# dcvan24/pivot-scheduling

Measured on AMD Instinct MI355X. Metric: task x host placement candidates scored/sec (HBM GB/s % peak) at 1/2/4/8 MI355X, higher is better.
Workload: dtype f64; 1 GPU; synthetic 1000000 hosts x 10000 ready tasks per round, 20 zones, cost_aware best-fit, one independent scenario per GPU; scenarios_per_gpu=1, tasks_per_round=10000, zones=20, policy=ca_bf, parallelism=scenario-sharded x1 (no data-path collective)

## Files before the change

pivot-scheduling_amd/csrc/pvt_capi.hip:

```cpp
#include <cstdarg>

#include "pvt_driver.h"
#include "pvt_opp.h"
#include "pvt_anchor.h"
#include "pvt_groups.h"
#include "pvt_meter.h"

int pvt::fail(pvt_ctx* c, int code, const char* fmt, ...) {
  char buf[512];
  va_list ap;
  va_start(ap, fmt);
  vsnprintf(buf, sizeof(buf), fmt, ap);
  va_end(ap);
  if (c) c->err = buf;
  return code;
}

int pvt::ensure(pvt_ctx* ctx, Buf& b, size_t bytes) {
  if (bytes == 0) bytes = 16;
  if (b.n >= bytes) return PVT_OK;
  const size_t want = std::max(bytes, b.n * 3 / 2);
  if (b.p) (void)hipFree(b.p);
  b.p = nullptr;
  b.n = 0;
// ... 182 lines not shown
extern "C" int pvt_reset_kstats(pvt_ctx* ctx) {
  if (!ctx) return PVT_EINVAL;
  (void)hipStreamSynchronize(ctx->stream);
  harvest(ctx);
  std::memset(ctx->ks, 0, sizeof(ctx->ks));
  ctx->kks.clear();
  return PVT_OK;
}
extern "C" int pvt_get_kstats(pvt_ctx* ctx, int kclass, pvt_kstats* out) {
  if (!ctx || !out || kclass < 0 || kclass >= PVT_K_COUNT) return PVT_EINVAL;
  (void)hipStreamSynchronize(ctx->stream);
  harvest(ctx);
  *out = ctx->ks[kclass];
  return PVT_OK;
}
extern "C" int pvt_get_kernel_kstats(pvt_ctx* ctx, const char* kernel, pvt_kstats* out) {
  if (!ctx || !kernel || !out) return PVT_EINVAL;
  (void)hipStreamSynchronize(ctx->stream);
  harvest(ctx);
  auto it = ctx->kks.find(kernel);
  if (it == ctx->kks.end()) std::memset(out, 0, sizeof(*out));
  else *out = it->second;
  return PVT_OK;
}
extern "C" int pvt_set_window(pvt_ctx* ctx, int tasks) {
  if (!ctx || tasks < 0) return PVT_EINVAL;
  ctx->window = std::min(tasks, MAX_WINDOW);
  return PVT_OK;
}
extern "C" int pvt_set_score_tw(pvt_ctx* ctx, int tw) {
  if (!ctx || (tw != 0 && tw != 2 && tw != 4)) return PVT_EINVAL;
  ctx->score_tw = tw;
  return PVT_OK;
}
extern "C" int pvt_set_pipeline(pvt_ctx* ctx, int on) {
  if (!ctx) return PVT_EINVAL;
  ctx->pipeline = on != 0;
  return PVT_OK;
}
extern "C" int pvt_set_epochs(pvt_ctx* ctx, int on) {
  if (!ctx) return PVT_EINVAL;
  ctx->epochs = on != 0;
  return PVT_OK;
}
extern "C" int pvt_epoch_stats(pvt_ctx* ctx, int64_t* epochs, int64_t* segments, int64_t* rejected) {
  if (!ctx) return PVT_EINVAL;
  if (epochs) *epochs = ctx->n_epochs;
  if (segments) *segments = ctx->n_segs;
  if (rejected) *rejected = ctx->n_rejected;
  return PVT_OK;
}
extern "C" int pvt_set_band(pvt_ctx* ctx, int32_t min_hosts) {
  if (!ctx || min_hosts < 0) return PVT_EINVAL;
  ctx->band_min = min_hosts;
  return PVT_OK;
}
extern "C" int pvt_set_zero_walk(pvt_ctx* ctx, int on) {
  if (!ctx) return PVT_EINVAL;
  ctx->zwalk = on != 0;
  return PVT_OK;
}
extern "C" int pvt_zero_walk_stats(pvt_ctx* ctx, int64_t* frontier_chains, int64_t* list_chains,
                                   int64_t* longest_chain) {
  if (!ctx) return PVT_EINVAL;
  if (frontier_chains) *frontier_chains = ctx->n_zchains;
  if (list_chains) *list_chains = ctx->n_gchains;
  if (longest_chain) *longest_chain = ctx->n_longest;
  return PVT_OK;
}
extern "C" int pvt_prologue_stats(pvt_ctx* ctx, int64_t* fast_chains) {
  if (!ctx) return PVT_EINVAL;
  if (fast_chains) *fast_chains = ctx->n_fastpro;
  return PVT_OK;
}
extern "C" int pvt_last_stats(pvt_ctx* ctx, int64_t* windows, int64_t* refills) {
  if (!ctx) return PVT_EINVAL;
  if (windows) *windows = ctx->windows;
  if (refills) *refills = ctx->refills;
  return PVT_OK;
}
extern "C" int pvt_debug_commit_stamps(pvt_ctx* ctx, uint64_t* out, int n) {
  if (!ctx || !out || n < 8) return PVT_EINVAL;
#ifdef PVT_STAMPS
  constexpr int NW = 32 + 4096;
  if (!ctx->stamps) {
    if (hipMalloc((void**)&ctx->stamps, sizeof(uint64_t) * NW) != hipSuccess) return PVT_ENOMEM;
    (void)hipMemset(ctx->stamps, 0, sizeof(uint64_t) * NW);
    std::memset(out, 0, sizeof(uint64_t) * std::min(n, NW));
    return PVT_OK;
  }
  if (hipMemcpy(out, ctx->stamps, sizeof(uint64_t) * std::min(n, NW), hipMemcpyDeviceToHost) != hipSuccess)
    return PVT_EHIP;
  return PVT_OK;
#else
  return PVT_EUNSUPPORTED;
#endif
}

extern "C" int pvt_debug_score_counts(pvt_ctx* ctx, uint64_t* out, int n, int reset) {
  if (!ctx || !out || n < 5) return PVT_EINVAL;
  (void)hipSetDevice(ctx->device);
  return pvt::score_diag(out, n, reset);
}

static_assert(PVT_MAX_ZONES == pvt::ZWIDE, "the public zone bound is the wide kernels' bound");
extern "C" int pvt_max_zones(void) { return PVT_MAX_ZONES; }

extern "C" const char* pvt_last_error(pvt_ctx* ctx) { return ctx ? ctx->err.c_str() : "null context"; }

int pvt::check_round(pvt_ctx* ctx, const pvt_round* r) {
  if (!r) return fail(ctx, PVT_EINVAL, "null round");
  if (r->reserved != 0) return fail(ctx, PVT_EINVAL, "reserved must be 0");
  if (r->n_hosts < 1 || r->n_tasks < 0 || r->n_zones < 1 || r->n_zones > PVT_MAX_ZONES)
    return fail(ctx, PVT_EINVAL, "bad sizes H=%d T=%d Z=%d (1 <= Z <= PVT_MAX_ZONES = %d)", r->n_hosts,
                r->n_tasks, r->n_zones, PVT_MAX_ZONES);
  if (r->mode < PVT_CA_FF || r->mode > PVT_VBP_BF) return fail(ctx, PVT_EINVAL, "bad mode %d", r->mode);
  if (!r->avail || !r->zone) return fail(ctx, PVT_EINVAL, "null host array");
  if (r->n_tasks > 0 && (!r->dem || !r->order || !r->placement))
    return fail(ctx, PVT_EINVAL, "null task array");
  if ((r->mode == PVT_CA_FF || r->mode == PVT_CA_BF) && (!r->cost || !r->bw))
    return fail(ctx, PVT_EINVAL, "cost_aware needs cost and bw");
  if (r->n_tasks > 0 && r->task_group && (r->n_groups < 1 || !r->group_anchor))
    return fail(ctx, PVT_EINVAL, "task_group needs n_groups >= 1 and group_anchor");
  if (r->mode == PVT_VBP_BF && !r->tiebreak) return fail(ctx, PVT_EINVAL, "vbp best-fit needs tiebreak");
  if (r->mode == PVT_OPP && !r->mt_state) return fail(ctx, PVT_EINVAL, "opportunistic needs mt_state");
  if (r->mode == PVT_CA_BF && r->decay && r->n_tasks > 0)
    return fail(ctx, PVT_EUNSUPPORTED, "cost_aware best-fit with host_decay (reference crashes, cost_aware.py:26,81)");
  return PVT_OK;
}

static const char* const CHK_NAMES[CHK_RULES + 1] = {
    "ok", "zone", "avail", "dem", "task_group", "group_anchor", "cost", "bw", "rt_bw", "decay",
    "tiebreak", "mt_state"};

int pvt::fail_check(pvt_ctx* ctx, int i, const pvt_check_report& p) {
  char where[32] = "";
  if (i >= 0) std::snprintf(where, sizeof(where), "round %d: ", i);
  return fail(ctx, PVT_EINVAL, "%scheck failed: rule %d (%s) at index %lld, value %.17g (%lld "
              "violating, mask 0x%x)", where, p.code, CHK_NAMES[p.code], (long long)p.index, p.value,
              (long long)p.count, (unsigned)p.mask);
}

static void check_mtpos(const pvt_round* r, pvt_check_report* p) {
  if (r->mode != PVT_OPP || !r->mt_state || !chk_bad_mtpos(r->mt_state[624])) return;
  p->mask |= 1 << PVT_CHK_MTPOS;
  if (p->code) return;
  p->code = PVT_CHK_MTPOS;
  p->index = 624;
  p->count = 1;
  p->value = (double)r->mt_state[624];
}

void pvt::check_host_arrays(const pvt_round* r, pvt_check_report* p) {
  check_on_host(check_describe(*r), p);
  check_mtpos(r, p);
}

static int run_checks(pvt_ctx* ctx, const pvt_round* rounds, int n, pvt_check_report* out,
                      bool host_mt) {
  for (int i = 0; i < n; i++) {
    int rc = check_round(ctx, &rounds[i]);
    if (rc) return rc;
  }
  HIPCHK(hipSetDevice(ctx->device));
  hipStream_t st = ctx->stream;
  std::vector<CheckRound>& cr = ctx->chk_host;
  cr.resize(n);
// ... 169 lines not shown
```

pivot-scheduling_amd/csrc/pvt_kernels.h:

```cpp
#pragma once
#include <hip/hip_runtime.h>
#include <hip/hip_ext.h>
#include <stdint.h>

namespace pvt {

struct TimedEvents {
  hipEvent_t a = nullptr, b = nullptr;
  bool armed = false;
  int used = 0, extra = 0;
};
extern thread_local TimedEvents g_timed;
#define PVT_LAUNCH(kernel, grid, block, shmem, stream, ...)                                         \
  do {                                                                                             \
    ::pvt::TimedEvents& te_ = ::pvt::g_timed;                                                      \
    if (te_.armed && te_.a) {                                                                      \
      hipExtLaunchKernelGGL(kernel, grid, block, shmem, stream, te_.a, te_.b, 0u, __VA_ARGS__);    \
      te_.a = nullptr;                                                                             \
      te_.used++;                                                                                  \
    } else {                                                                                       \
      if (te_.armed) te_.extra++;                                                                  \
      hipLaunchKernelGGL(kernel, grid, block, shmem, stream, __VA_ARGS__);                         \
    }                                                                                              \
  } while (0)
// ... 413 lines not shown
              resident_switches(32, 1025) == resident_switches(32, 1024), "32 holds at every size");
static_assert(resident_switches(64 + (12 << 8), 1024) == ResidentSwitches{0, 0, 0, 0, 1, 1, 1, 12} &&
              resident_switches(64 + (12 << 8), 1025) == resident_switches(64 + (12 << 8), 1024),
              "64 and the list minimum hold at every size");
static_assert(resident_switches(2, 1024) == ResidentSwitches{1, 0, 1, 1, 1, 1, 0, 0}, "2: rotated walker");
struct ResidentArgs {
  const void* rounds;
  uint32_t* mt;
  int Zb;
  int Tpad;
  uint64_t* stamps;
  ResidentSwitches sw;
};
size_t resident_lds_bytes(int Zb, int Tpad, const ResidentSwitches& sw);
void resident_shape(int maxH, int* waves, int* hpl);
void launch_resident(int mode, int waves, int hpl, int n, size_t lds, const ResidentArgs& a,
                     hipStream_t st);
hipError_t resident_init_attrs();
constexpr int RES_WIDE_MAX_HPL = 8;
constexpr int RES_WIDE_MAX_HOSTS = 4 * WAVE * RES_WIDE_MAX_HPL;
void launch_resident_wide(int mode, int hpl, int n, size_t lds, const ResidentArgs& a, hipStream_t st);
hipError_t resident_wide_init_attrs();

struct FusedRound {
  int64_t out_lo, out_hi, in_lo, in_hi;
  int64_t desc;
  int32_t items, pad;
};
struct FusedArgs {
  const char* hmap;
  char* dev;
  int64_t o_rounds;
  int64_t o_ka, o_kg;
  ResidentArgs ra;
};
size_t fused_pre_lds_bytes();
void launch_fused(int mode, int hpl, int n, size_t lds, const FusedArgs& F, hipStream_t st);
void launch_fused_wide(int mode, int hpl, int n, size_t lds, const FusedArgs& F, hipStream_t st);
size_t commit_lds_bytes();
hipError_t init_kernel_attrs();
constexpr int GSORT_MAX = 4096;
void launch_group_hist(const int32_t* tg, int T, int G, int32_t* cnt, hipStream_t st);
constexpr int PREP_T_MAX = 65536;
constexpr int GAGG_MAX = 4096;
struct PrepArgs {
  const int32_t* tg;
  int T, G;
  const int32_t* ganc;
  const double* cost;
  const double* bw;
  int Z, nz2;
  const double* dem;
  int sort_tasks;
  int32_t* placement;
  int32_t* off;
  int32_t* hcnt;
  int32_t* hgan;
  double* hcst;
  double* csum;
  double* bsum;
  uint64_t* skey;
  int32_t* sidx;
  int32_t* hflag;
  int32_t seq;
};
void launch_order_prep(const PrepArgs& a, hipStream_t st, hipEvent_t counted = nullptr,
                       bool scatter = true);
constexpr int GCOMPACT_MAX = 64;
struct GatherOut {
  int32_t* ord;
  double* dem_ord;
  int32_t* anc_ord;
  int32_t* grp_ord;
  int32_t* order_out;
  const double* avail;
  int H;
  double* hmin;
  uint64_t* stamps;
  const int32_t* zone;
  struct ZoneWindows* zwin;
  struct GroupCert* gcert;
};
static_assert(GC_SUB * 64 == GSORT_MAX, "a group record holds every sub-batch of a sorted group");
void launch_group_sort_gather(const PrepArgs& a, const GatherOut& o, hipStream_t st);
void launch_upload(const void* src_mapped, void* dst, size_t bytes, hipStream_t st);
void launch_restore_hosts(double* avail, const double* avail0, int H, const int32_t* hosts, int n,
                          hipStream_t st);
void launch_group_stage(const int32_t* cnt, int G, const int32_t* ganc, const double* cost, int nz2,
                        int32_t* off, int32_t* hcnt, int32_t* hgan, double* hcst, hipStream_t st);
void launch_group_scatter(const int32_t* tg, const uint64_t* keys, int T, int G, int32_t* cursor,
                          uint64_t* skey, int32_t* sidx, hipStream_t st);
void launch_group_sort(const int32_t* off, int G, const uint64_t* skey, const int32_t* sidx,
                       int32_t* ord, hipStream_t st);
void launch_iota(int32_t* out, int n, hipStream_t st);
void launch_gather_tasks(const double* dem, const int32_t* ord, const int32_t* task_group,
                         const int32_t* group_anchor, int T, double* dem_ord, int32_t* anc_ord,
                         int32_t* grp_ord, hipStream_t st, int G = 0x7fffffff,
                         int32_t* order_out = nullptr);

}
```

pivot-scheduling_amd/csrc/pvt_kernels.hip:

```cpp
#include <hip/hip_runtime.h>
#include <algorithm>
#include <stdint.h>
#include <stdlib.h>

#include "pvt_device.h"
#include "pvt_kernels.h"
#include "pvt_zwin_dev.h"
#include "pvt_list.h"

namespace pvt {

#ifdef PVT_DIAG
__device__ unsigned long long g_score_diag[8];
#endif

template <int MODE, int TWP>
__global__ __launch_bounds__(256) void score_kernel(ScoreArgs A) {
  constexpr bool WIDE = TWP < 0;
  constexpr int TW = WIDE ? -TWP : TWP;
  constexpr bool STRICT = (MODE != CA_BF);
  constexpr int ZL = (MODE == CA_BF && !WIDE) ? ZMAX : 1;
  __shared__ double s_lim[WPB][TW][ZL];
  __shared__ double s_rad[WPB][TW][ZL];
  __shared__ double s_c[WPB][TW][ZL];
// ... 996 lines not shown
  __threadfence_system();
  if (A.hflag) {
    __syncthreads();
    if (t == 0) {
      __hip_atomic_store(A.hflag, A.seq, __ATOMIC_RELEASE, __HIP_MEMORY_SCOPE_SYSTEM);
    }
  }
}
__global__ __launch_bounds__(1024) void order_count_kernel(PrepArgs A) {
  __shared__ int32_t cnt[GAGG_MAX + 1];
  order_count_body(A, cnt);
}

__global__ __launch_bounds__(1024) void order_scatter_kernel(PrepArgs A) {
  __shared__ int32_t cur[GAGG_MAX];
  __shared__ int32_t wsum[16];
  __shared__ int32_t carry;
  const int t = threadIdx.x, lane = t & 63, wave = t >> 6;
  const int T = A.T, G = A.G;
  if (t == 0) carry = 0;
  if (A.placement)
    for (int i = t; i < T; i += 1024) A.placement[i] = -1;
  if (A.csum)
    for (int i = t; i < A.Z * A.Z; i += 1024) {
      const int a = i / A.Z, z = i - a * A.Z;
      A.csum[i] = A.cost[a * A.Z + z] + A.cost[z * A.Z + a];
      A.bsum[i] = A.bw[a * A.Z + z] + A.bw[z * A.Z + a];
    }
  __syncthreads();
  for (int g0 = 0; g0 < G; g0 += 1024) {
    const int g = g0 + t;
    const int v = g < G ? A.off[g] : 0;
    int x = v;
#pragma unroll
    for (int o = 1; o < 64; o <<= 1) {
      const int y = __shfl_up(x, o);
      if (lane >= o) x += y;
    }
    if (lane == 63) wsum[wave] = x;
    __syncthreads();
    int pre = carry;
    for (int w = 0; w < wave; w++) pre += wsum[w];
    if (g < G) { A.off[g] = pre + x - v; cur[g] = pre + x - v; }
    __syncthreads();
    if (t == 1023) carry = pre + x;
    __syncthreads();
  }
  if (t == 0) A.off[G] = carry;
  constexpr int PS = 8;
  for (int i0 = 0; i0 < T; i0 += 1024 * PS) {
    int gv[PS];
    double dv[PS][4];
#pragma unroll
    for (int u = 0; u < PS; u++) {
      const int i = i0 + u * 1024 + t;
      gv[u] = i < T ? A.tg[i] : -1;
      if (A.sort_tasks && i < T) {
        dv[u][0] = A.dem[i]; dv[u][1] = A.dem[(size_t)T + i];
        dv[u][2] = A.dem[2 * (size_t)T + i]; dv[u][3] = A.dem[3 * (size_t)T + i];
      }
    }
#pragma unroll
    for (int u = 0; u < PS; u++) {
      const int i = i0 + u * 1024 + t;
      const int g = gv[u];
      if (i >= T || g < 0 || g >= G) continue;
      uint64_t key = 0;
      if (A.sort_tasks) {
        const double n = __builtin_sqrt(norm2_seq(dv[u][0], dv[u][1], dv[u][2], dv[u][3]));
        key = ~(uint64_t)__double_as_longlong(n);
      }
      const int pos = atomicAdd(&cur[g], 1);
      A.skey[pos] = key;
      A.sidx[pos] = i;
    }
  }
}
void launch_order_prep(const PrepArgs& a, hipStream_t st, hipEvent_t counted, bool scatter) {
  PVT_LAUNCH(order_count_kernel, dim3(1), dim3(1024), 0, st, a);
  if (counted) (void)hipEventRecord(counted, st);
  if (scatter) PVT_LAUNCH(order_scatter_kernel, dim3(1), dim3(1024), 0, st, a);
}

__device__ void lds_sort_pairs(uint64_t* k, int32_t* v, int n) {
  const int tid = threadIdx.x;
  if (n <= 128) {
    int r = 0;
    int32_t vi = 0;
    if (tid < n) {
      const uint64_t ki = k[tid];
      vi = v[tid];
      for (int j = 0; j < n; j++) {
        const uint64_t kj = k[j];
        r += (kj < ki || (kj == ki && v[j] < vi)) ? 1 : 0;
      }
    }
    __syncthreads();
    if (tid < n) v[r] = vi;
    __syncthreads();
    return;
  }
  int P = 2;
  while (P < n) P <<= 1;
  constexpr int EMAX = GSORT_MAX / 1024;
  const int E = (P + 1023) >> 10;
  uint64_t rk[EMAX];
  int32_t rv[EMAX];
#pragma unroll
  for (int m = 0; m < EMAX; m++) {
    const int i = m * 1024 + tid;
    rk[m] = (m < E && i < n) ? k[i] : ~0ull;
    rv[m] = (m < E && i < n) ? v[i] : (0x40000000 + i);
  }
  __syncthreads();
  const int P64 = min(P, 64);
  for (int size = 2; size <= P64; size <<= 1) {
    for (int stride = size >> 1; stride > 0 && (tid & ~63) < P; stride >>= 1) {
#pragma unroll
      for (int m = 0; m < EMAX; m++) {
        if (m >= E) continue;
        const int i = m * 1024 + tid;
        const uint32_t klo = (uint32_t)rk[m], khi = (uint32_t)(rk[m] >> 32);
        const uint64_t pk = ((uint64_t)(uint32_t)__shfl_xor((int)khi, stride) << 32) |
                            (uint32_t)__shfl_xor((int)klo, stride);
        const int32_t pv = __shfl_xor(rv[m], stride);
        const bool up = size == P64 || (i & size) == 0, low = (i & stride) == 0;
        const uint64_t kl = low ? rk[m] : pk, kh = low ? pk : rk[m];
        const int32_t vl = low ? rv[m] : pv, vh = low ? pv : rv[m];
        const bool gt = kl > kh || (kl == kh && vl > vh);
        if (gt == up) { rk[m] = pk; rv[m] = pv; }
      }
    }
  }
  if (P <= 64) {
#pragma unroll
    for (int m = 0; m < EMAX; m++) {
      const int i = m * 1024 + tid;
      if (m < E && i < n) v[i] = rv[m];
    }
    __syncthreads();
    return;
  }
  __shared__ uint64_t k2[GSORT_MAX];
  __shared__ int32_t v2[GSORT_MAX];
#pragma unroll
  for (int m = 0; m < EMAX; m++) {
    const int i = m * 1024 + tid;
    if (m < E && i < P) { k[i] = rk[m]; v[i] = rv[m]; }
  }
  __syncthreads();
  uint64_t* ka = k;
  int32_t* va = v;
  uint64_t* kb = k2;
  int32_t* vb = v2;
  for (int w = 64; w < P; w <<= 1) {
#pragma unroll
    for (int m = 0; m < EMAX; m++) {
      const int i = m * 1024 + tid;
      if (m >= E || i >= P) continue;
      const uint64_t key = ka[i];
      const int32_t val = va[i];
      const int base = i & ~(2 * w - 1), off = i - base;
      const bool left = off < w;
      const int ob = left ? base + w : base;
      int lo = 0, len = w;
      while (len > 0) {
        const int half = len >> 1, mid = lo + half;
        const uint64_t km = ka[ob + mid];
        const bool below = km < key || (km == key && va[ob + mid] < val);
        lo = below ? mid + 1 : lo;
        len = below ? len - half - 1 : half;
      }
      const int dest = base + (left ? off : off - w) + lo;
      kb[dest] = key;
      vb[dest] = val;
    }
    __syncthreads();
    uint64_t* tk = ka; ka = kb; kb = tk;
    int32_t* tv = va; va = vb; vb = tv;
  }
  if (va != v) {
    for (int i = tid; i < n; i += 1024) v[i] = va[i];
    __syncthreads();
  }
}

__global__ __launch_bounds__(1024) void group_sort_kernel(const int32_t* off, const uint64_t* skey,
                                                          const int32_t* sidx, int32_t* ord) {
  __shared__ uint64_t k[GSORT_MAX];
  __shared__ int32_t v[GSORT_MAX];
  const int a = off[blockIdx.x], n = off[blockIdx.x + 1] - a, tid = threadIdx.x;
  if (n <= 0 || n > GSORT_MAX) return;
  for (int i = tid; i < n; i += blockDim.x) { k[i] = skey[a + i]; v[i] = sidx[a + i]; }
  __syncthreads();
  lds_sort_pairs(k, v, n);
  for (int i = tid; i < n; i += blockDim.x) ord[a + i] = v[i];
}

__device__ void zone_window_block(const PrepArgs& A, const GatherOut& O, int j, int32_t* lds) {
  __shared__ uint32_t am[ZMAX], reach[ZMAX], gm_s;
  __shared__ int32_t cnt[2][16], nw_s;
  const int tid = threadIdx.x, Z = A.Z;
  ZoneWindows* W = O.zwin;
  if (tid < ZMAX) am[tid] = 0;
  if (tid == 0) { gm_s = 0; nw_s = 0; }
  __syncthreads();
  for (int i = tid; i < Z * Z; i += 1024) {
    const int a = i / Z, z = i - a * Z;
    if (A.cost[a * Z + z] + A.cost[z * Z + a] == 0.0) atomicOr(&am[a], 1u << z);
  }
  for (int g = tid; g < A.G; g += 1024) {
    const int a = A.ganc[g];
    if (a >= 0 && a < Z) atomicOr(&gm_s, 1u << a);
  }
  __syncthreads();
  if (tid < Z) reach[tid] = am[tid] | (1u << tid);
  __syncthreads();
  for (int it = 0; it < 5; it++) {
    uint32_t r = 0;
    if (tid < Z) {
      r = reach[tid];
      for (uint32_t m = r; m; m &= m - 1) r |= reach[__builtin_ctz(m)];
    }
    __syncthreads();
    if (tid < Z) reach[tid] = r;
    __syncthreads();
  }
  const uint32_t comp = reach[j];
  uint32_t U = 0;
  if ((comp & ((1u << j) - 1u)) == 0)
    for (uint32_t m = comp & gm_s; m; m &= m - 1) U |= am[__builtin_ctz(m)];
  if (tid == 0) W->U[j] = U;
  if (U == 0) return;
  int32_t* wid = lds;
  int32_t* wz = lds + ZW_M;
  compact_zone_window_t<ZW_M, 1024, 2>(O.zone, Z, U, 0, O.H, wid, wz, cnt, &nw_s);
  const int n = nw_s;
  ZoneWindow& w = W->w[j];
  bool bad = false;
  for (int p = tid; p < n; p += 1024) {
    const int h = wid[p];
    w.id[p] = h;
    w.z[p] = wz[p];
#pragma unroll
    for (int r = 0; r < 4; r++) {
      const double x = O.avail[(size_t)r * O.H + h];
      bad |= !(__builtin_fabs(x) <= 0x1p500);
      w.a[r][p] = x;
    }
  }
  bad = __syncthreads_or(bad);
  if (tid == 0) { w.n = n; w.bad = bad ? 1 : 0; }
}

#ifdef PVT_STAMPS
__device__ __forceinline__ uint64_t gstamp() {
  uint64_t t;
  __builtin_amdgcn_sched_barrier(0);
  asm volatile("s_memtime %0\n\ts_waitcnt lgkmcnt(0)" : "=s"(t)::"memory");
  __builtin_amdgcn_sched_barrier(0);
  return t;
}
#define GSTAMP(k) do { if (g == 0 && tid == 0 && O.stamps) { const uint64_t t_ = gstamp(); gph[k] = t_ - gtl; gtl = t_; } } while (0)
#else
#define GSTAMP(k) do {} while (0)
#endif

__global__ __launch_bounds__(1024) void group_sort_gather_kernel(PrepArgs A, GatherOut O) {
  __shared__ uint64_t k[GSORT_MAX];
  __shared__ int32_t v[GSORT_MAX];
  __shared__ int32_t fill, below_s;
  static_assert(sizeof(k) >= sizeof(int32_t) * (GCOMPACT_MAX + 1), "count table in k");
  if (blockIdx.x == 0) {
    order_count_body(A, reinterpret_cast<int32_t*>(k));
    return;
  }
  const int g = blockIdx.x - 1, tid = threadIdx.x, lane = tid & 63;
  const int T = A.T;
#ifdef PVT_STAMPS
  uint64_t gph[4] = {0, 0, 0, 0}, gtl = 0;
  if (g == 0 && tid == 0) gtl = gstamp();
#endif
  const int nmin = O.hmin ? ZW_MIN_PARTS : 0;
  if (g >= A.G + nmin) {
    zone_window_block(A, O, g - A.G - nmin, reinterpret_cast<int32_t*>(k));
    return;
  }
  if (g >= A.G) {
    __shared__ double red[16][4];
    const int pb = g - A.G, wave = tid >> 6;
    double m[4] = {DINF, DINF, DINF, DINF};
    constexpr int STEP = ZW_MIN_PARTS * 1024;
    for (int h0 = pb * 1024 + tid; h0 < O.H; h0 += 4 * STEP) {
      double x[4][4];
#pragma unroll
      for (int j = 0; j < 4; j++) {
        const int h = h0 + j * STEP;
#pragma unroll
        for (int r = 0; r < 4; r++) x[j][r] = h < O.H ? O.avail[(size_t)r * O.H + h] : DINF;
      }
#pragma unroll
      for (int j = 0; j < 4; j++)
#pragma unroll
        for (int r = 0; r < 4; r++) m[r] = fmin(m[r], x[j][r]);
    }
#pragma unroll
    for (int r = 0; r < 4; r++) {
      for (int off = 32; off > 0; off >>= 1) m[r] = fmin(m[r], __shfl_xor(m[r], off));
      if (lane == 0) red[wave][r] = m[r];
    }
    __syncthreads();
    if (tid < 4) {
      double x = red[0][tid];
      for (int w = 1; w < 16; w++) x = fmin(x, red[w][tid]);
      O.hmin[pb * 4 + tid] = x;
    }
    return;
  }
  if (g == 0 && A.csum)
    for (int i = tid; i < A.Z * A.Z; i += 1024) {
      const int a = i / A.Z, z = i - a * A.Z;
      A.csum[i] = A.cost[a * A.Z + z] + A.cost[z * A.Z + a];
      A.bsum[i] = A.bw[a * A.Z + z] + A.bw[z * A.Z + a];
    }
  if (tid == 0) { fill = 0; below_s = 0; }
  __syncthreads();
  GSTAMP(0);
  const uint64_t below = (lane == 0) ? 0ull : (~0ull >> (64 - lane));
  constexpr int PB = 8;
  for (int i0 = 0; i0 < T; i0 += 1024 * PB) {
    int gv[PB];
#pragma unroll
    for (int u = 0; u < PB; u++) {
      const int i = i0 + u * 1024 + tid;
      gv[u] = i < T ? A.tg[i] : -1;
    }
    uint64_t bal[PB];
    int tot = 0, lt = 0;
#pragma unroll
    for (int u = 0; u < PB; u++) {
      const int i = i0 + u * 1024 + tid;
      const bool mine = gv[u] == g;
      if (mine && A.placement) A.placement[i] = -1;
      bal[u] = __ballot(mine);
      tot += __popcll(bal[u]);
      lt += __popcll(__ballot(gv[u] >= 0 && gv[u] < g));
    }
    if (lane == 0 && lt) atomicAdd(&below_s, lt);
    if (tot == 0) continue;
    int b = 0;
    if (lane == 0) b = atomicAdd(&fill, tot);
    b = __shfl(b, 0);
    if (b + tot > GSORT_MAX) continue;
#pragma unroll
    for (int u = 0; u < PB; u++) {
      if (gv[u] == g) v[b + __popcll(bal[u] & below)] = i0 + u * 1024 + tid;
      b += __popcll(bal[u]);
    }
  }
  __syncthreads();
  const int n = fill;
  if (n > GSORT_MAX && tid == 0 && O.gcert) { O.gcert[g].bad = 2; O.gcert[g].n = n; }
  if (n > GSORT_MAX || n <= 0) return;
  for (int q = tid; q < n; q += 1024) {
    uint64_t key = 0;
    if (A.sort_tasks) {
      const int i = v[q];
      const double nn = __builtin_sqrt(norm2_seq(A.dem[i], A.dem[(size_t)T + i],
                                                 A.dem[2 * (size_t)T + i], A.dem[3 * (size_t)T + i]));
      key = ~(uint64_t)__double_as_longlong(nn);
    }
    k[q] = key;
  }
  __syncthreads();
  GSTAMP(1);
  lds_sort_pairs(k, v, n);
  GSTAMP(2);
  const int a = below_s;
  const int32_t anc = A.ganc[g];
  GroupCert* const gc = O.gcert ? O.gcert + g : nullptr;
  const int wave = __builtin_amdgcn_readfirstlane(tid >> 6);
  double gmx[4] = {-DINF, -DINF, -DINF, -DINF}, gmn[4] = {DINF, DINF, DINF, DINF};
  bool gbad = false;
  for (int i0 = 0; i0 < n; i0 += 1024) {
    const int i = i0 + tid;
    double d[4] = {0.0, 0.0, 0.0, 0.0};
    if (i < n) {
      const int p = a + i, t = v[i];
      O.ord[p] = t;
      if (O.order_out) O.order_out[p] = t;
      double* o = O.dem_ord + (size_t)p * 4;
      d[0] = A.dem[t]; d[1] = A.dem[(size_t)T + t]; d[2] = A.dem[2 * (size_t)T + t]; d[3] = A.dem[3 * (size_t)T + t];
      o[0] = d[0]; o[1] = d[1]; o[2] = d[2]; o[3] = d[3];
      O.anc_ord[p] = anc;
      O.grp_ord[p] = g;
    }
    if (gc && i0 + wave * 64 < n) {
#pragma unroll
      for (int r = 0; r < 4; r++) {
        const double f = readlane_d(d[r], 0);
        const double x = i < n ? d[r] : f;
        gbad |= !(__builtin_fabs(x) <= 0x1p500);
        gmx[r] = fmax(gmx[r], x);
        double m = f;
        if (__ballot(__double_as_longlong(x) != __double_as_longlong(f)) != 0) m = wave_min_d(x);
        gmn[r] = fmin(gmn[r], m);
        if (lane == 0) gc->smin[(i0 >> 6) + wave][r] = m;
      }
    }
  }
  if (gc) {
    double* red = reinterpret_cast<double*>(k);
#pragma unroll
    for (int r = 0; r < 4; r++) {
      const double f = readlane_d(gmx[r], 0);
      double m = f;
      if (__ballot(__double_as_longlong(gmx[r]) != __double_as_longlong(f)) != 0) m = wave_max_d(gmx[r]);
      if (lane == 0) { red[wave * 8 + r] = m; red[wave * 8 + 4 + r] = gmn[r]; }
    }
    gbad = __syncthreads_or(gbad);
    if (tid < 8) {
      double x = red[tid];
      for (int w = 1; w < 16; w++) x = tid < 4 ? fmax(x, red[w * 8 + tid]) : fmin(x, red[w * 8 + tid]);
      if (tid < 4) gc->mx[tid] = x; else gc->mn[tid - 4] = x;
    }
    if (tid == 0) { gc->bad = gbad ? 1 : 0; gc->n = n; }
  }
#ifdef PVT_STAMPS
  __syncthreads();
  GSTAMP(3);
  if (g == 0 && tid == 0 && O.stamps)
    for (int q = 0; q < 4; q++) atomicAdd((unsigned long long*)&O.stamps[16 + q], (unsigned long long)gph[q]);
#endif
}
void launch_group_sort_gather(const PrepArgs& a, const GatherOut& o, hipStream_t st) {
  const int extra = (o.hmin ? ZW_MIN_PARTS : 0) + (o.zwin ? a.Z : 0);
  PVT_LAUNCH(group_sort_gather_kernel, dim3(1 + a.G + extra), dim3(1024), 0, st, a, o);
}
void launch_group_sort(const int32_t* off, int G, const uint64_t* skey, const int32_t* sidx,
                       int32_t* ord, hipStream_t st) {
  PVT_LAUNCH(group_sort_kernel, dim3(G), dim3(1024), 0, st, off, skey, sidx, ord);
}

__global__ __launch_bounds__(256) void restore_hosts_kernel(double* avail, const double* avail0, int H,
                                                            const int32_t* hosts, int n) {
  const int i = blockIdx.x * 256 + threadIdx.x;
  if (i >= n) return;
  const int h = hosts[i];
  if (h < 0 || h >= H) return;
#pragma unroll
  for (int r = 0; r < 4; r++) avail[(size_t)r * H + h] = avail0[(size_t)r * H + h];
}
void launch_restore_hosts(double* avail, const double* avail0, int H, const int32_t* hosts, int n,
                          hipStream_t st) {
  if (n > 0) PVT_LAUNCH(restore_hosts_kernel, dim3((n + 255) / 256), dim3(256), 0, st, avail, avail0, H, hosts, n);
}

__global__ __launch_bounds__(256) void upload_kernel(const int4* src, int4* dst, int n16) {
  for (int i = blockIdx.x * 256 + threadIdx.x; i < n16; i += gridDim.x * 256) dst[i] = src[i];
}
void launch_upload(const void* src_mapped, void* dst, size_t bytes, hipStream_t st) {
  const int n16 = (int)((bytes + 15) / 16);
  if (n16 <= 0) return;
  const int blocks = std::min(64, (n16 + 255) / 256);
  PVT_LAUNCH(upload_kernel, dim3(blocks), dim3(256), 0, st,
                     reinterpret_cast<const int4*>(src_mapped), reinterpret_cast<int4*>(dst), n16);
}

__global__ void iota_kernel(int32_t* out, int n) {
  const int i = blockIdx.x * blockDim.x + threadIdx.x;
  if (i < n) out[i] = i;
}
void launch_iota(int32_t* out, int n, hipStream_t st) {
  PVT_LAUNCH(iota_kernel, dim3((n + 255) / 256), dim3(256), 0, st, out, n);
}

__global__ void gather_tasks_kernel(const double* dem, const int32_t* ord, const int32_t* tg,
                                    const int32_t* ga, int T, double* dem_ord, int32_t* anc_ord,
                                    int32_t* grp_ord, int G, int32_t* order_out) {
  const int p = blockIdx.x * blockDim.x + threadIdx.x;
  if (p >= T) return;
  const int t = ord[p];
  if (order_out) order_out[p] = t;
  double* o = dem_ord + (size_t)p * 4;
  o[0] = dem[t]; o[1] = dem[(size_t)T + t]; o[2] = dem[2 * (size_t)T + t]; o[3] = dem[3 * (size_t)T + t];
  if (anc_ord) anc_ord[p] = (tg && ga && tg[t] >= 0 && tg[t] < G) ? ga[tg[t]] : 0;
  if (grp_ord) grp_ord[p] = tg ? tg[t] : 0;
}
void launch_gather_tasks(const double* dem, const int32_t* ord, const int32_t* task_group,
                         const int32_t* group_anchor, int T, double* dem_ord, int32_t* anc_ord,
                         int32_t* grp_ord, hipStream_t st, int G, int32_t* order_out) {
  PVT_LAUNCH(gather_tasks_kernel, dim3((T + 255) / 256), dim3(256), 0, st, dem, ord,
                     task_group, group_anchor, T, dem_ord, anc_ord, grp_ord, G, order_out);
}

}
```

pivot-scheduling_amd/csrc/pvt_round.hip:

```cpp
#include <hipcub/hipcub.hpp>

#include <limits>

#include "pvt_driver.h"
#include "pvt_opp.h"
#include "pvt_groups.h"

static constexpr size_t SEG_ENTRIES_MAX = (size_t)MAX_WINDOW * MAX_SEG * KL;
static int choose_segments(int H, int nt, int mode, int force_tw, bool epoch, int force_S, int Z) {
  const int tw = score_tasks_per_wave(mode, H, force_tw, Z);
  const int task_waves = (nt + tw - 1) / tw;
  int S = (4096 + task_waves - 1) / task_waves;
  if (mode == PVT_VBP_BF) S = std::min(S, 16);
  if (mode == PVT_CA_BF && epoch) S = 4;
  if (force_S > 0) S = force_S;
  S = std::min(S, std::max(1, H / 4096));
  S = std::min(S, std::max(MAX_SEG, (int)(SEG_ENTRIES_MAX / ((size_t)nt * KL))));
  S = std::max(1, std::min(S, 256));
  if (S >= 8) S = S / 8 * 8;
  return S;
}
static constexpr int KSCAN_DEPTH = 256;
static constexpr int KPREFIX_MIN = 1024;
double pvt::bytes_per_candidate(int mode) {
// ... 7 lines not shown
    if (n >= (1u << 18)) {
      HIPCHK(hipStreamSynchronize(ctx->stream));
      if (__atomic_load_n(f, __ATOMIC_ACQUIRE) == seq) return PVT_OK;
      return fail(ctx, PVT_EHIP, "%s: kernel finished without its flag", what);
    }
    if ((n & 4095) == 0) {
      const hipError_t e = hipStreamQuery(ctx->stream);
      if (e == hipSuccess) {
        if (__atomic_load_n(f, __ATOMIC_ACQUIRE) == seq) return PVT_OK;
        return fail(ctx, PVT_EHIP, "%s: kernel finished without its flag", what);
      }
      if (e != hipErrorNotReady) return fail(ctx, PVT_EHIP, "%s: %s", what, hipGetErrorString(e));
    }
  }
}
static int wait_stage_flag(pvt_ctx* ctx) {
  return wait_host_flag(ctx, ctx->flag_host, ctx->flag_seq, "grouped order");
}

static int build_order_radix(pvt_ctx* ctx, const pvt_round* r, int32_t** ord_out);
static int build_order(pvt_ctx* ctx, const pvt_round* r, int32_t** ord_out, bool* pending,
                       double* hmin = nullptr, bool* hmin_done = nullptr,
                       ZoneWindows* zwin = nullptr) {
  *pending = false;
  if (hmin_done) *hmin_done = false;
  ctx->rs.stage_flag = false;
  const int T = r->n_tasks;
  hipStream_t st = ctx->stream;
  ENSURE(ctx->ord, sizeof(int32_t) * T);
  ENSURE(ctx->ord2, sizeof(int32_t) * T);
  int32_t* cur = P<int32_t>(ctx->ord);
  const bool grouped = r->task_group != nullptr && r->n_groups > 1;
  RoundState& R = ctx->rs;
  R.ginfo = false;
  R.zpre = false;
  R.gcert = false;
  if (grouped && r->n_groups <= (1 << 20)) {
    const int G = r->n_groups;
    const bool fused = T <= PREP_T_MAX && G <= GAGG_MAX;
    if (!fused) {
      ENSURE(ctx->gcnt, sizeof(int32_t) * (G + 1));
      HIPCHK(hipMemsetAsync(ctx->gcnt.p, 0, sizeof(int32_t) * (G + 1), st));
      launch_group_hist(r->task_group, T, G, P<int32_t>(ctx->gcnt), st);
    }
    const bool ca = r->mode == PVT_CA_FF || r->mode == PVT_CA_BF;
    const size_t nz2 = ca ? (size_t)r->n_zones * r->n_zones : 0;
    const size_t need = sizeof(double) * nz2 + sizeof(int32_t) * (2 * (size_t)G + 1);
    if (ctx->gstage_cap < need) {
      if (ctx->gstage) (void)hipHostFree(ctx->gstage);
      ctx->gstage = nullptr;
      ctx->gstage_cap = 0;
      HIPCHK(hipHostMalloc(&ctx->gstage, need));
      ctx->gstage_cap = need;
    }
    ENSURE(ctx->goff, sizeof(int32_t) * 2 * (G + 1));
    void* dstage = nullptr;
    HIPCHK(hipHostGetDevicePointer(&dstage, ctx->gstage, 0));
    double* dcst = reinterpret_cast<double*>(dstage);
    int32_t* dcnt = reinterpret_cast<int32_t*>(dcst + nz2);
    ENSURE(ctx->gskey, sizeof(uint64_t) * T);
    ENSURE(ctx->gsidx, sizeof(int32_t) * T);
    if (fused) {
      if (ca) {
        ENSURE(ctx->csum, sizeof(double) * r->n_zones * r->n_zones);
        ENSURE(ctx->bsum, sizeof(double) * r->n_zones * r->n_zones);
      }
      PrepArgs pa{r->task_group, T, G, r->group_anchor, r->cost, r->bw, r->n_zones, (int)nz2,
                  r->dem, r->sort_tasks ? 1 : 0, r->placement, P<int32_t>(ctx->goff), dcnt,
                  dcnt + G + 1, dcst, ca ? P<double>(ctx->csum) : nullptr,
                  ca ? P<double>(ctx->bsum) : nullptr, P<uint64_t>(ctx->gskey), P<int32_t>(ctx->gsidx),
                  nullptr, 0};
      R.prep_fused = true;
      if (G <= GCOMPACT_MAX) {
        pa.hflag = ctx->flag_hdev;
        pa.seq = ++ctx->flag_seq;
        R.stage_flag = true;
        const bool zw = hmin && zwin && ca && r->n_zones <= ZMAX;
        const bool gc = zw && ctx->t_chain_cert;
        if (gc) ENSURE(ctx->gcert, sizeof(GroupCert) * (size_t)GCOMPACT_MAX);
        launch_group_sort_gather(pa, GatherOut{cur, P<double>(ctx->dem_ord), P<int32_t>(ctx->anc_ord),
                                               P<int32_t>(ctx->grp_ord), r->order, r->avail,
                                               r->n_hosts, hmin, ctx->stamps, r->zone,
                                               zw ? zwin : nullptr,
                                               gc ? P<GroupCert>(ctx->gcert) : nullptr}, st);
        if (hmin_done) *hmin_done = hmin != nullptr;
        R.zpre = zw;
        R.gcert = gc;
        R.gathered = true;
        R.ginfo = ca;
        *pending = true;
        *ord_out = cur;
        return PVT_OK;
      }
      launch_order_prep(pa, st, ctx->ev_stage);
    } else {
      launch_group_stage(P<int32_t>(ctx->gcnt), G, r->group_anchor, r->cost, (int)nz2,
                         P<int32_t>(ctx->goff), dcnt, dcnt + G + 1, dcst, st);
      HIPCHK(hipGetLastError());
      const uint64_t* keys = nullptr;
      if (r->sort_tasks) {
        ENSURE(ctx->keys64a, sizeof(uint64_t) * T);
        launch_norm_keys(r->dem, T, nullptr, P<uint64_t>(ctx->keys64a), st);
        keys = P<uint64_t>(ctx->keys64a);
      }
      launch_group_scatter(r->task_group, keys, T, G, P<int32_t>(ctx->goff) + G + 1,
                           P<uint64_t>(ctx->gskey), P<int32_t>(ctx->gsidx), st);
      HIPCHK(hipEventRecord(ctx->ev_stage, st));
    }
    launch_group_sort(P<int32_t>(ctx->goff), G, P<uint64_t>(ctx->gskey), P<int32_t>(ctx->gsidx),
                      cur, st);
    R.ginfo = ca;
    *pending = true;
    *ord_out = cur;
    return PVT_OK;
  }
  return build_order_radix(ctx, r, ord_out);
}

static int build_order_check(pvt_ctx* ctx, const pvt_round* r, bool* redo) {
  RoundState& R = ctx->rs;
  const int G = r->n_groups;
  const bool ca = r->mode == PVT_CA_FF || r->mode == PVT_CA_BF;
  const size_t nz2 = ca ? (size_t)r->n_zones * r->n_zones : 0;
  const double* cst = reinterpret_cast<const double*>(ctx->gstage);
  const int32_t* cnt = reinterpret_cast<const int32_t*>(cst + nz2);
  const int32_t* gan = cnt + G + 1;
  R.gcnt.assign(cnt, cnt + G + 1);
  R.ga_host.assign(gan, gan + G);
  R.cost_host.assign(cst, cst + nz2);
  if (R.gcnt[G] != 0) return fail(ctx, PVT_EINVAL, "task_group out of range");
  int mx = 0;
  for (int g = 0; g < G; g++) mx = std::max(mx, R.gcnt[g]);
  *redo = mx > GSORT_MAX;
  return PVT_OK;
}

static int build_order_radix(pvt_ctx* ctx, const pvt_round* r, int32_t** ord_out) {
  const int T = r->n_tasks;
  hipStream_t st = ctx->stream;
  int32_t* cur = P<int32_t>(ctx->ord);
  int32_t* alt = P<int32_t>(ctx->ord2);
  const bool grouped = r->task_group != nullptr && r->n_groups > 1;
  launch_iota(cur, T, st);
  if (r->sort_tasks) {
    ENSURE(ctx->keys64a, sizeof(uint64_t) * T);
    ENSURE(ctx->keys64b, sizeof(uint64_t) * T);
    launch_norm_keys(r->dem, T, nullptr, P<uint64_t>(ctx->keys64a), st);
    size_t tmp = 0;
    HIPCHK(hipcub::DeviceRadixSort::SortPairs(nullptr, tmp, P<uint64_t>(ctx->keys64a),
                                              P<uint64_t>(ctx->keys64b), cur, alt, T, 0, 64, st));
    ENSURE(ctx->sorttmp, tmp);
    HIPCHK(hipcub::DeviceRadixSort::SortPairs(ctx->sorttmp.p, tmp, P<uint64_t>(ctx->keys64a),
                                              P<uint64_t>(ctx->keys64b), cur, alt, T, 0, 64, st));
    std::swap(cur, alt);
  }
  if (grouped) {
    ENSURE(ctx->keys32a, sizeof(uint32_t) * T);
    ENSURE(ctx->keys32b, sizeof(uint32_t) * T);
    launch_group_keys(r->task_group, cur, T, P<uint32_t>(ctx->keys32a), st);
    int bits = 1;
    while ((1 << bits) < r->n_groups && bits < 31) bits++;
    size_t tmp = 0;
    HIPCHK(hipcub::DeviceRadixSort::SortPairs(nullptr, tmp, P<uint32_t>(ctx->keys32a),
                                              P<uint32_t>(ctx->keys32b), cur, alt, T, 0, bits, st));
    ENSURE(ctx->sorttmp, tmp);
    HIPCHK(hipcub::DeviceRadixSort::SortPairs(ctx->sorttmp.p, tmp, P<uint32_t>(ctx->keys32a),
                                              P<uint32_t>(ctx->keys32b), cur, alt, T, 0, bits, st));
// ... 784 lines not shown
```

Measured before the change: 60280 billion candidates/s.

## Size host-min blocks to CU count and cache group demand rows in LDS

The group sort/gather kernel now orders blocks as count, groups, zone windows, then host-min partitions. The number of host-min blocks is derived from the CU count rather than fixed, with wider unrolling when fewer blocks are used and unused partial slots filled with infinity. Group demand rows are staged in LDS during key computation so the gather reads them back instead of re-reading global memory. The sort also pads to a multiple of 64 instead of a power of two, and fine-grained stamp instrumentation is added. In exchange it uses more LDS per block and may reduce occupancy.

```diff
diff --git a/pivot-scheduling_amd/csrc/pvt_capi.hip b/pivot-scheduling_amd/csrc/pvt_capi.hip
--- a/pivot-scheduling_amd/csrc/pvt_capi.hip
+++ b/pivot-scheduling_amd/csrc/pvt_capi.hip
@@ -288,7 +288,8 @@
 extern "C" int pvt_debug_commit_stamps(pvt_ctx* ctx, uint64_t* out, int n) {
   if (!ctx || !out || n < 8) return PVT_EINVAL;
 #ifdef PVT_STAMPS
-  constexpr int NW = 32 + 4096;
+  constexpr int NW = pvt::ORD_ST_END;
+  static_assert(pvt::ORD_ST_BASE == 32 + 4096, "the order launch's stamps follow the resident rounds");
   if (!ctx->stamps) {
     if (hipMalloc((void**)&ctx->stamps, sizeof(uint64_t) * NW) != hipSuccess) return PVT_ENOMEM;
     (void)hipMemset(ctx->stamps, 0, sizeof(uint64_t) * NW);
diff --git a/pivot-scheduling_amd/csrc/pvt_kernels.h b/pivot-scheduling_amd/csrc/pvt_kernels.h
--- a/pivot-scheduling_amd/csrc/pvt_kernels.h
+++ b/pivot-scheduling_amd/csrc/pvt_kernels.h
@@ -519,7 +519,14 @@
   struct GroupCert* gcert;
 };
 static_assert(GC_SUB * 64 == GSORT_MAX, "a group record holds every sub-batch of a sorted group");
-void launch_group_sort_gather(const PrepArgs& a, const GatherOut& o, hipStream_t st);
+constexpr int ORD_ST_BASE = 32 + 4096;
+constexpr int ORD_ST_BLOCKS = 512, ORD_ST_GPH = 16, ORD_ST_WPH = 4;
+constexpr int ORD_ST_BLK = ORD_ST_BASE + 8;
+constexpr int ORD_ST_GRP = ORD_ST_BLK + 2 * ORD_ST_BLOCKS;
+constexpr int ORD_ST_WIN = ORD_ST_GRP + GCOMPACT_MAX * ORD_ST_GPH;
+constexpr int ORD_ST_END = ORD_ST_WIN + ZMAX * ORD_ST_WPH;
+constexpr int ORD_MINB_FLOOR = 32;
+void launch_group_sort_gather(const PrepArgs& a, const GatherOut& o, int cus, hipStream_t st);
 void launch_upload(const void* src_mapped, void* dst, size_t bytes, hipStream_t st);
 void launch_restore_hosts(double* avail, const double* avail0, int H, const int32_t* hosts, int n,
                           hipStream_t st);
diff --git a/pivot-scheduling_amd/csrc/pvt_kernels.hip b/pivot-scheduling_amd/csrc/pvt_kernels.hip
--- a/pivot-scheduling_amd/csrc/pvt_kernels.hip
+++ b/pivot-scheduling_amd/csrc/pvt_kernels.hip
@@ -1102,7 +1102,12 @@
   if (scatter) PVT_LAUNCH(order_scatter_kernel, dim3(1), dim3(1024), 0, st, a);
 }
 
-__device__ void lds_sort_pairs(uint64_t* k, int32_t* v, int n) {
+#ifdef PVT_STAMPS
+#define SSTAMP(q) do { if (st && tid == 0) st[q] = wall_clock64(); } while (0)
+#else
+#define SSTAMP(q) do {} while (0)
+#endif
+__device__ void lds_sort_pairs(uint64_t* k, int32_t* v, int n, uint64_t* st = nullptr) {
   const int tid = threadIdx.x;
   if (n <= 128) {
     int r = 0;
@@ -1120,31 +1125,29 @@
     __syncthreads();
     return;
   }
-  int P = 2;
-  while (P < n) P <<= 1;
+  const int N = (n + 63) & ~63;
   constexpr int EMAX = GSORT_MAX / 1024;
-  const int E = (P + 1023) >> 10;
   uint64_t rk[EMAX];
   int32_t rv[EMAX];
 #pragma unroll
   for (int m = 0; m < EMAX; m++) {
     const int i = m * 1024 + tid;
-    rk[m] = (m < E && i < n) ? k[i] : ~0ull;
-    rv[m] = (m < E && i < n) ? v[i] : (0x40000000 + i);
-  }
-  __syncthreads();
-  const int P64 = min(P, 64);
-  for (int size = 2; size <= P64; size <<= 1) {
-    for (int stride = size >> 1; stride > 0 && (tid & ~63) < P; stride >>= 1) {
+    rk[m] = i < n ? k[i] : ~0ull;
+    rv[m] = i < n ? v[i] : (0x40000000 + i);
+  }
+  __syncthreads();
+  SSTAMP(0);
+  for (int size = 2; size <= 64; size <<= 1) {
+    for (int stride = size >> 1; stride > 0; stride >>= 1) {
 #pragma unroll
       for (int m = 0; m < EMAX; m++) {
-        if (m >= E) continue;
         const int i = m * 1024 + tid;
+        if ((i & ~63) >= N) continue;
         const uint32_t klo = (uint32_t)rk[m], khi = (uint32_t)(rk[m] >> 32);
         const uint64_t pk = ((uint64_t)(uint32_t)__shfl_xor((int)khi, stride) << 32) |
                             (uint32_t)__shfl_xor((int)klo, stride);
         const int32_t pv = __shfl_xor(rv[m], stride);
-        const bool up = size == P64 || (i & size) == 0, low = (i & stride) == 0;
+        const bool up = size == 64 || (i & size) == 0, low = (i & stride) == 0;
         const uint64_t kl = low ? rk[m] : pk, kh = low ? pk : rk[m];
         const int32_t vl = low ? rv[m] : pv, vh = low ? pv : rv[m];
         const bool gt = kl > kh || (kl == kh && vl > vh);
@@ -1152,38 +1155,31 @@
       }
     }
   }
-  if (P <= 64) {
-#pragma unroll
-    for (int m = 0; m < EMAX; m++) {
-      const int i = m * 1024 + tid;
-      if (m < E && i < n) v[i] = rv[m];
-    }
-    __syncthreads();
-    return;
-  }
+  SSTAMP(1);
   __shared__ uint64_t k2[GSORT_MAX];
   __shared__ int32_t v2[GSORT_MAX];
 #pragma unroll
   for (int m = 0; m < EMAX; m++) {
     const int i = m * 1024 + tid;
-    if (m < E && i < P) { k[i] = rk[m]; v[i] = rv[m]; }
-  }
-  __syncthreads();
+    if (i < N) { k[i] = rk[m]; v[i] = rv[m]; }
+  }
+  __syncthreads();
+  SSTAMP(2);
   uint64_t* ka = k;
   int32_t* va = v;
   uint64_t* kb = k2;
   int32_t* vb = v2;
-  for (int w = 64; w < P; w <<= 1) {
+  for (int w = 64; w < N; w <<= 1) {
 #pragma unroll
     for (int m = 0; m < EMAX; m++) {
       const int i = m * 1024 + tid;
-      if (m >= E || i >= P) continue;
+      if (i >= N) continue;
       const uint64_t key = ka[i];
       const int32_t val = va[i];
       const int base = i & ~(2 * w - 1), off = i - base;
       const bool left = off < w;
       const int ob = left ? base + w : base;
-      int lo = 0, len = w;
+      int lo = 0, len = max(min(w, N - ob), 0);
       while (len > 0) {
         const int half = len >> 1, mid = lo + half;
         const uint64_t km = ka[ob + mid];
@@ -1217,6 +1213,14 @@
   for (int i = tid; i < n; i += blockDim.x) ord[a + i] = v[i];
 }
 
+#ifdef PVT_STAMPS
+#define GSTAMP(k) do { if (tid == 0 && O.stamps) O.stamps[ORD_ST_GRP + g * ORD_ST_GPH + 1 + (k)] = wall_clock64(); } while (0)
+#define WSTAMP(k) do { if (tid == 0 && O.stamps) O.stamps[ORD_ST_WIN + j * ORD_ST_WPH + (k)] = wall_clock64(); } while (0)
+#else
+#define GSTAMP(k) do {} while (0)
+#define WSTAMP(k) do {} while (0)
+#endif
+
 __device__ void zone_window_block(const PrepArgs& A, const GatherOut& O, int j, int32_t* lds) {
   __shared__ uint32_t am[ZMAX], reach[ZMAX], gm_s;
   __shared__ int32_t cnt[2][16], nw_s;
@@ -1251,11 +1255,13 @@
   if ((comp & ((1u << j) - 1u)) == 0)
     for (uint32_t m = comp & gm_s; m; m &= m - 1) U |= am[__builtin_ctz(m)];
   if (tid == 0) W->U[j] = U;
+  WSTAMP(0);
   if (U == 0) return;
   int32_t* wid = lds;
   int32_t* wz = lds + ZW_M;
   compact_zone_window_t<ZW_M, 1024, 2>(O.zone, Z, U, 0, O.H, wid, wz, cnt, &nw_s);
   const int n = nw_s;
+  WSTAMP(1);
   ZoneWindow& w = W->w[j];
   bool bad = false;
   for (int p = tid; p < n; p += 1024) {
@@ -1271,25 +1277,49 @@
   }
   bad = __syncthreads_or(bad);
   if (tid == 0) { w.n = n; w.bad = bad ? 1 : 0; }
-}
-
-#ifdef PVT_STAMPS
-__device__ __forceinline__ uint64_t gstamp() {
-  uint64_t t;
-  __builtin_amdgcn_sched_barrier(0);
-  asm volatile("s_memtime %0\n\ts_waitcnt lgkmcnt(0)" : "=s"(t)::"memory");
-  __builtin_amdgcn_sched_barrier(0);
-  return t;
-}
-#define GSTAMP(k) do { if (g == 0 && tid == 0 && O.stamps) { const uint64_t t_ = gstamp(); gph[k] = t_ - gtl; gtl = t_; } } while (0)
-#else
-#define GSTAMP(k) do {} while (0)
-#endif
-
-__global__ __launch_bounds__(1024) void group_sort_gather_kernel(PrepArgs A, GatherOut O) {
+  WSTAMP(2);
+}
+
+template <int U>
+__device__ __forceinline__ void host_min_block(const GatherOut& O, int pb, int nb) {
+  __shared__ double red[16][4];
+  const int tid = threadIdx.x, lane = tid & 63, wave = tid >> 6;
+  double m[4] = {DINF, DINF, DINF, DINF};
+  const size_t step = (size_t)nb * 1024, H = (size_t)O.H;
+  for (size_t h0 = (size_t)pb * 1024 + tid; h0 < H; h0 += U * step) {
+    double x[U][4];
+#pragma unroll
+    for (int j = 0; j < U; j++) {
+      const size_t h = h0 + j * step;
+#pragma unroll
+      for (int r = 0; r < 4; r++) x[j][r] = h < H ? O.avail[(size_t)r * H + h] : DINF;
+    }
+#pragma unroll
+    for (int j = 0; j < U; j++)
+#pragma unroll
+      for (int r = 0; r < 4; r++) m[r] = fmin(m[r], x[j][r]);
+  }
+#pragma unroll
+  for (int r = 0; r < 4; r++) {
+    for (int off = 32; off > 0; off >>= 1) m[r] = fmin(m[r], __shfl_xor(m[r], off));
+    if (lane == 0) red[wave][r] = m[r];
+  }
+  __syncthreads();
+  if (tid < 4) {
+    double x = red[0][tid];
+    for (int w = 1; w < 16; w++) x = fmin(x, red[w][tid]);
+    O.hmin[pb * 4 + tid] = x;
+    for (int q = pb + nb; q < ZW_MIN_PARTS; q += nb) O.hmin[q * 4 + tid] = DINF;
+  }
+}
+
+__device__ __forceinline__ void group_sort_gather_block(const PrepArgs& A, const GatherOut& O) {
   __shared__ uint64_t k[GSORT_MAX];
   __shared__ int32_t v[GSORT_MAX];
   __shared__ int32_t fill, below_s;
+  constexpr int GROW_MAX = 1024;
+  __shared__ double rows[GROW_MAX][4];
+  static_assert(PREP_T_MAX <= (1 << 16) && GROW_MAX <= (1 << 12), "(task << 12) | slot below 2^30");
   static_assert(sizeof(k) >= sizeof(int32_t) * (GCOMPACT_MAX + 1), "count table in k");
   if (blockIdx.x == 0) {
     order_count_body(A, reinterpret_cast<int32_t*>(k));
@@ -1297,46 +1327,26 @@
   }
   const int g = blockIdx.x - 1, tid = threadIdx.x, lane = tid & 63;
   const int T = A.T;
+  const int nwin = O.zwin ? A.Z : 0;
+  const int nmin = (int)gridDim.x - 1 - A.G - nwin;
 #ifdef PVT_STAMPS
-  uint64_t gph[4] = {0, 0, 0, 0}, gtl = 0;
-  if (g == 0 && tid == 0) gtl = gstamp();
+  if (g == 0 && tid == 0 && O.stamps) {
+    uint64_t* hd = O.stamps + ORD_ST_BASE;
+    hd[0] = gridDim.x; hd[1] = A.G; hd[2] = 1 + A.G + nwin; hd[3] = nmin;
+    hd[4] = 1 + A.G; hd[5] = nwin;
+  }
 #endif
-  const int nmin = O.hmin ? ZW_MIN_PARTS : 0;
-  if (g >= A.G + nmin) {
-    zone_window_block(A, O, g - A.G - nmin, reinterpret_cast<int32_t*>(k));
+  if (g >= A.G + nwin) {
+    const int pb = g - A.G - nwin;
+    if (nmin < ZW_MIN_PARTS) host_min_block<8>(O, pb, nmin);
+    else host_min_block<4>(O, pb, nmin);
     return;
   }
   if (g >= A.G) {
-    __shared__ double red[16][4];
-    const int pb = g - A.G, wave = tid >> 6;
-    double m[4] = {DINF, DINF, DINF, DINF};
-    constexpr int STEP = ZW_MIN_PARTS * 1024;
-    for (int h0 = pb * 1024 + tid; h0 < O.H; h0 += 4 * STEP) {
-      double x[4][4];
-#pragma unroll
-      for (int j = 0; j < 4; j++) {
-        const int h = h0 + j * STEP;
-#pragma unroll
-        for (int r = 0; r < 4; r++) x[j][r] = h < O.H ? O.avail[(size_t)r * O.H + h] : DINF;
-      }
-#pragma unroll
-      for (int j = 0; j < 4; j++)
-#pragma unroll
-        for (int r = 0; r < 4; r++) m[r] = fmin(m[r], x[j][r]);
-    }
-#pragma unroll
-    for (int r = 0; r < 4; r++) {
-      for (int off = 32; off > 0; off >>= 1) m[r] = fmin(m[r], __shfl_xor(m[r], off));
-      if (lane == 0) red[wave][r] = m[r];
-    }
-    __syncthreads();
-    if (tid < 4) {
-      double x = red[0][tid];
-      for (int w = 1; w < 16; w++) x = fmin(x, red[w][tid]);
-      O.hmin[pb * 4 + tid] = x;
-    }
+    zone_window_block(A, O, g - A.G, reinterpret_cast<int32_t*>(k));
     return;
   }
+  GSTAMP(0);
   if (g == 0 && A.csum)
     for (int i = tid; i < A.Z * A.Z; i += 1024) {
       const int a = i / A.Z, z = i - a * A.Z;
@@ -1345,10 +1355,11 @@
     }
   if (tid == 0) { fill = 0; below_s = 0; }
   __syncthreads();
-  GSTAMP(0);
-  const uint64_t below = (lane == 0) ? 0ull : (~0ull >> (64 - lane));
+  GSTAMP(1);
+  const uint64_t below =(lane == 0) ? 0ull : (~0ull >> (64 - lane));
   constexpr int PB = 8;
   for (int i0 = 0; i0 < T; i0 += 1024 * PB) {
+    GSTAMP(2 + min(i0 / (1024 * PB), 3));
     int gv[PB];
 #pragma unroll
     for (int u = 0; u < PB; u++) {
@@ -1379,23 +1390,39 @@
     }
   }
   __syncthreads();
+  GSTAMP(6);
   const int n = fill;
+#ifdef PVT_STAMPS
+  if (tid == 0 && O.stamps) O.stamps[ORD_ST_GRP + g * ORD_ST_GPH] = (uint64_t)n;
+#endif
   if (n > GSORT_MAX && tid == 0 && O.gcert) { O.gcert[g].bad = 2; O.gcert[g].n = n; }
   if (n > GSORT_MAX || n <= 0) return;
+  const bool held = n <= GROW_MAX;
   for (int q = tid; q < n; q += 1024) {
     uint64_t key = 0;
-    if (A.sort_tasks) {
-      const int i = v[q];
-      const double nn = __builtin_sqrt(norm2_seq(A.dem[i], A.dem[(size_t)T + i],
-                                                 A.dem[2 * (size_t)T + i], A.dem[3 * (size_t)T + i]));
-      key = ~(uint64_t)__double_as_longlong(nn);
+    const int i = v[q];
+    if (A.sort_tasks || held) {
+      const double d0 = A.dem[i], d1 = A.dem[(size_t)T + i], d2 = A.dem[2 * (size_t)T + i],
+                   d3 = A.dem[3 * (size_t)T + i];
+      if (held) {
+        rows[q][0] = d0; rows[q][1] = d1; rows[q][2] = d2; rows[q][3] = d3;
+        v[q] = (i << 12) | q;
+      }
+      if (A.sort_tasks) {
+        const double nn = __builtin_sqrt(norm2_seq(d0, d1, d2, d3));
+        key = ~(uint64_t)__double_as_longlong(nn);
+      }
     }
     k[q] = key;
   }
   __syncthreads();
-  GSTAMP(1);
+  GSTAMP(7);
+#ifdef PVT_STAMPS
+  lds_sort_pairs(k, v, n, O.stamps ? O.stamps + ORD_ST_GRP + g * ORD_ST_GPH + 12 : nullptr);
+#else
   lds_sort_pairs(k, v, n);
-  GSTAMP(2);
+#endif
+  GSTAMP(8);
   const int a = below_s;
   const int32_t anc = A.ganc[g];
   GroupCert* const gc = O.gcert ? O.gcert + g : nullptr;
@@ -1406,11 +1433,16 @@
     const int i = i0 + tid;
     double d[4] = {0.0, 0.0, 0.0, 0.0};
     if (i < n) {
-      const int p = a + i, t = v[i];
+      const int p = a + i, e = v[i], t = held ? e >> 12 : e;
       O.ord[p] = t;
       if (O.order_out) O.order_out[p] = t;
       double* o = O.dem_ord + (size_t)p * 4;
-      d[0] = A.dem[t]; d[1] = A.dem[(size_t)T + t]; d[2] = A.dem[2 * (size_t)T + t]; d[3] = A.dem[3 * (size_t)T + t];
+      if (held) {
+        const double* row = rows[e & 4095];
+        d[0] = row[0]; d[1] = row[1]; d[2] = row[2]; d[3] = row[3];
+      } else {
+        d[0] = A.dem[t]; d[1] = A.dem[(size_t)T + t]; d[2] = A.dem[2 * (size_t)T + t]; d[3] = A.dem[3 * (size_t)T + t];
+      }
       o[0] = d[0]; o[1] = d[1]; o[2] = d[2]; o[3] = d[3];
       O.anc_ord[p] = anc;
       O.grp_ord[p] = g;
@@ -1429,6 +1461,10 @@
       }
     }
   }
+#ifdef PVT_STAMPS
+  __syncthreads();
+  GSTAMP(9);
+#endif
   if (gc) {
     double* red = reinterpret_cast<double*>(k);
 #pragma unroll
@@ -1448,14 +1484,24 @@
   }
 #ifdef PVT_STAMPS
   __syncthreads();
-  GSTAMP(3);
-  if (g == 0 && tid == 0 && O.stamps)
-    for (int q = 0; q < 4; q++) atomicAdd((unsigned long long*)&O.stamps[16 + q], (unsigned long long)gph[q]);
+  GSTAMP(10);
 #endif
 }
-void launch_group_sort_gather(const PrepArgs& a, const GatherOut& o, hipStream_t st) {
-  const int extra = (o.hmin ? ZW_MIN_PARTS : 0) + (o.zwin ? a.Z : 0);
-  PVT_LAUNCH(group_sort_gather_kernel, dim3(1 + a.G + extra), dim3(1024), 0, st, a, o);
+__global__ __launch_bounds__(1024) void group_sort_gather_kernel(PrepArgs A, GatherOut O) {
+#ifdef PVT_STAMPS
+  const bool st = threadIdx.x == 0 && O.stamps && blockIdx.x < ORD_ST_BLOCKS;
+  if (st) O.stamps[ORD_ST_BLK + 2 * blockIdx.x] = wall_clock64();
+#endif
+  group_sort_gather_block(A, O);
+#ifdef PVT_STAMPS
+  __syncthreads();
+  if (st) O.stamps[ORD_ST_BLK + 2 * blockIdx.x + 1] = wall_clock64();
+#endif
+}
+void launch_group_sort_gather(const PrepArgs& a, const GatherOut& o, int cus, hipStream_t st) {
+  const int fixed = 1 + a.G + (o.zwin ? a.Z : 0);
+  const int nmin = o.hmin ? std::max(std::min(ZW_MIN_PARTS, cus - fixed), ORD_MINB_FLOOR) : 0;
+  PVT_LAUNCH(group_sort_gather_kernel, dim3(fixed + nmin), dim3(1024), 0, st, a, o);
 }
 void launch_group_sort(const int32_t* off, int G, const uint64_t* skey, const int32_t* sidx,
                        int32_t* ord, hipStream_t st) {
diff --git a/pivot-scheduling_amd/csrc/pvt_round.hip b/pivot-scheduling_amd/csrc/pvt_round.hip
--- a/pivot-scheduling_amd/csrc/pvt_round.hip
+++ b/pivot-scheduling_amd/csrc/pvt_round.hip
@@ -113,7 +113,8 @@
                                                P<int32_t>(ctx->grp_ord), r->order, r->avail,
                                                r->n_hosts, hmin, ctx->stamps, r->zone,
                                                zw ? zwin : nullptr,
-                                               gc ? P<GroupCert>(ctx->gcert) : nullptr}, st);
+                                               gc ? P<GroupCert>(ctx->gcert) : nullptr},
+                                 ctx->n_cus, st);
         if (hmin_done) *hmin_done = hmin != nullptr;
         R.zpre = zw;
         R.gcert = gc;
```

New measurement: 60470 billion candidates/s, median of 2. About the same (+0.3%).
